# chintha/U-VIP-SLAM

Hardware: AMD Instinct MI355X
Metric: frames/sec ORB extract+match, 640x512 @1000 kp (higher is better)
Workload: dtype u8; 1 GPU; BASELINE.json configs[2]: 1xMI355X per rank, batch=256 synthetic 640x512 mono frames (+1 halo frame: the neighbouring rank's first), 1000 feats, 8 levels, fastTh 20, FullDetect extract + all-pairs 256-bit Hamming knn-2 of consecutive frames, HBM-resident I/O; batch_per_gpu=256, pipeline_depth=2, input_batches_in_rotation=4, fast_mode=adaptive

## Files before the change

u-vip-slam_amd/csrc/hamming.hip:

```cpp
#include "common.hpp"

namespace uvo {

constexpr int HM_TILE = 128;

__device__ __forceinline__ int popc256(const uint4& qa, const uint4& qb, const uint4& ta, const uint4& tb) {
  int d = __popc(qa.x ^ ta.x);
  d += __popc(qa.y ^ ta.y);
  d += __popc(qa.z ^ ta.z);
  d += __popc(qa.w ^ ta.w);
  d += __popc(qb.x ^ tb.x);
  d += __popc(qb.y ^ tb.y);
  d += __popc(qb.z ^ tb.z);
  d += __popc(qb.w ^ tb.w);
  return d;
}

__device__ __forceinline__ int clamp_count(int n, int cap) { return n < 0 ? 0 : (n > cap ? cap : n); }

__global__ __launch_bounds__(256) void k_knn2(const uint8_t* __restrict__ q, const int32_t* __restrict__ nq_arr, int nq_fixed, int q_stride,
                                              const uint8_t* __restrict__ t, const int32_t* __restrict__ nt_arr, int nt_fixed, int t_stride,
                                              const uint8_t* __restrict__ mask, int out_stride, int32_t* __restrict__ idx0,
                                              uint16_t* __restrict__ d0, int32_t* __restrict__ idx1, uint16_t* __restrict__ d1) {
  __shared__ uint4 s_t[HM_TILE * 2];
  const int pair = blockIdx.y;
  const int nq = nq_arr ? clamp_count(nq_arr[pair], q_stride < out_stride ? q_stride : out_stride) : nq_fixed;
  const int nt = nt_arr ? clamp_count(nt_arr[pair], t_stride < 65535 ? t_stride : 65535) : nt_fixed;
  const int qi = blockIdx.x * 256 + threadIdx.x;
  if (blockIdx.x * 256 >= nq) return;
  const uint4* Q = reinterpret_cast<const uint4*>(q + (int64_t)pair * q_stride * 32);
  const uint4* T = reinterpret_cast<const uint4*>(t + (int64_t)pair * t_stride * 32);
  const bool live = qi < nq;
  uint4 qa = make_uint4(0, 0, 0, 0), qb = qa;
  if (live) {
    qa = Q[2 * qi];
    qb = Q[2 * qi + 1];
  }
  uint32_t k0 = 0xFFFFFFFFu, k1 = 0xFFFFFFFFu;
  const uint8_t* mrow = mask ? mask + (int64_t)qi * nt : nullptr;
  for (int base = 0; base < nt; base += HM_TILE) {
    const int cnt = nt - base < HM_TILE ? nt - base : HM_TILE;
    __syncthreads();
    if ((int)threadIdx.x < 2 * cnt) s_t[threadIdx.x] = T[2 * base + threadIdx.x];
    __syncthreads();
    if (live) {
      for (int j = 0; j < cnt; ++j) {
        const uint32_t d = (uint32_t)popc256(qa, qb, s_t[2 * j], s_t[2 * j + 1]);
        uint32_t key = (d << 16) | (uint32_t)(base + j);
        if (mrow && !mrow[base + j]) key = 0xFFFFFFFFu;
        const uint32_t lo = min(k0, key);
        k1 = min(k1, max(k0, key));
        k0 = lo;
      }
    }
  }
  if (live) {
    const int64_t o = (int64_t)pair * out_stride + qi;
    idx0[o] = k0 == 0xFFFFFFFFu ? -1 : (int32_t)(k0 & 0xffffu);
    d0[o] = k0 == 0xFFFFFFFFu ? (uint16_t)0xFFFF : (uint16_t)(k0 >> 16);
    idx1[o] = k1 == 0xFFFFFFFFu ? -1 : (int32_t)(k1 & 0xffffu);
    d1[o] = k1 == 0xFFFFFFFFu ? (uint16_t)0xFFFF : (uint16_t)(k1 >> 16);
  }
}

typedef int v4i __attribute__((ext_vector_type(4)));
typedef int v16i __attribute__((ext_vector_type(16)));
constexpr int KM_ROW = 272;

__device__ __forceinline__ uint32_t spread4(uint32_t t) { return (__umul24(t & 0xfu, 0x00204081u)) & 0x01010101u; }
__device__ __forceinline__ v4i spread16(uint32_t x) {
  v4i r;
  r.x = (int)spread4(x), r.y = (int)spread4(x >> 4), r.z = (int)spread4(x >> 8), r.w = (int)spread4(x >> 12);
  return r;
}
__device__ __forceinline__ uint32_t spread4_ff(uint32_t t) {
  const uint32_t b = spread4(t);
  return (b << 8) - b;
}
__device__ __forceinline__ v4i spread16_ff(uint32_t x) {
  v4i r;
  r.x = (int)spread4_ff(x), r.y = (int)spread4_ff(x >> 4), r.z = (int)spread4_ff(x >> 8), r.w = (int)spread4_ff(x >> 12);
  return r;
}

__device__ __forceinline__ int med3_i32(int a, int b, int c) {
  int r;
  asm("v_med3_i32 %0, %1, %2, %3" : "=v"(r) : "v"(a), "v"(b), "v"(c));
  return r;
}

#ifndef UVO_OCC_KNN
#define UVO_OCC_KNN 6
#endif
__global__ __launch_bounds__(256, UVO_OCC_KNN) void k_knn2_mfma(const uint8_t* __restrict__ q, const int32_t* __restrict__ nq_arr, int nq_fixed, int q_stride,
                                                   const uint8_t* __restrict__ t, const int32_t* __restrict__ nt_arr, int nt_fixed, int t_stride,
                                                   int out_stride, int32_t* __restrict__ idx0, uint16_t* __restrict__ d0,
                                                   int32_t* __restrict__ idx1, uint16_t* __restrict__ d1) {
  __shared__ __attribute__((aligned(16))) uint8_t s_exp[32 * KM_ROW];
  __shared__ __attribute__((aligned(16))) int32_t s_key[32];
  const int pair = blockIdx.y;
  const int nq = nq_arr ? clamp_count(nq_arr[pair], q_stride < out_stride ? q_stride : out_stride) : nq_fixed;
  const int nt = nt_arr ? clamp_count(nt_arr[pair], t_stride < 65535 ? t_stride : 65535) : nt_fixed;
  if (blockIdx.x * 128 >= nq) return;
  const int lane = threadIdx.x & 63, wv = wave_in_block();
  const int r = lane & 31, h = lane >> 5;
  const int qi = blockIdx.x * 128 + wv * 32 + r;
  const uint32_t* Q = reinterpret_cast<const uint32_t*>(q + (int64_t)pair * q_stride * 32);
  const uint32_t* T = reinterpret_cast<const uint32_t*>(t + (int64_t)pair * t_stride * 32);
  v4i bq[8];
  int popq = 0;
#pragma unroll
  for (int s = 0; s < 8; ++s) {
    const uint32_t w = qi < nq ? Q[(int64_t)qi * 8 + s] : 0u;
    popq += __popc(w);
    bq[s] = spread16_ff(w >> (16 * h));
  }
  int k0 = 0x7fffffff, k1 = 0x7fffffff;
  const int erow = threadIdx.x >> 3, ec = threadIdx.x & 7;
  uint32_t wnext = erow < nt ? T[(int64_t)erow * 8 + ec] : 0u;
  for (int base = 0; base < nt; base += 32) {
    __syncthreads();
    {
      const int tr = base + erow;
      const uint32_t w = wnext;
      wnext = tr + 32 < nt ? T[(int64_t)(tr + 32) * 8 + ec] : 0u;
      v4i* dst = reinterpret_cast<v4i*>(s_exp + erow * KM_ROW + ec * 32);
      dst[0] = spread16(w), dst[1] = spread16(w >> 16);
      int pc = __popc(w);
      pc += __shfl_xor(pc, 1, 64);
      pc += __shfl_xor(pc, 2, 64);
      pc += __shfl_xor(pc, 4, 64);
      if (ec == 0) s_key[erow] = tr < nt ? ((pc << 16) | tr) : 0x7fff0000;
    }
    __syncthreads();
    v16i acc = {0, 0, 0, 0, 0, 0, 0, 0, 0, 0, 0, 0, 0, 0, 0, 0};
    const uint8_t* arow = s_exp + r * KM_ROW + 16 * h;
#pragma unroll
    for (int s = 0; s < 8; ++s) {
      const v4i a = *reinterpret_cast<const v4i*>(arow + 32 * s);
      acc = __builtin_amdgcn_mfma_i32_32x32x32_i8(a, bq[s], acc, 0, 0, 0);
    }
#pragma unroll
    for (int g = 0; g < 4; ++g) {
      const v4i kb = *reinterpret_cast<const v4i*>(&s_key[8 * g + 4 * h]);
      const int kbv[4] = {kb.x, kb.y, kb.z, kb.w};
#pragma unroll
      for (int e = 0; e < 4; ++e) {
        const int key = (int)(((uint32_t)acc[4 * g + e] << 17) + (uint32_t)kbv[e]);
        k1 = med3_i32(k0, k1, key);
        k0 = min(k0, key);
      }
    }
  }
  const int o0 = __shfl_xor(k0, 32, 64), o1 = __shfl_xor(k1, 32, 64);
  const int m0 = min(k0, o0), m1 = min(max(k0, o0), min(k1, o1));
  if (h == 0 && qi < nq) {
    const int64_t o = (int64_t)pair * out_stride + qi;
    const bool v0 = m0 < 0x7fff0000, v1 = m1 < 0x7fff0000;
    idx0[o] = v0 ? (m0 & 0xffff) : -1;
    d0[o] = v0 ? (uint16_t)((m0 >> 16) + popq) : (uint16_t)0xFFFF;
    idx1[o] = v1 ? (m1 & 0xffff) : -1;
    d1[o] = v1 ? (uint16_t)((m1 >> 16) + popq) : (uint16_t)0xFFFF;
  }
}

__global__ __launch_bounds__(256) void k_matrix(const uint8_t* __restrict__ q, int nq, const uint8_t* __restrict__ t, int nt,
                                                uint16_t* __restrict__ dist) {
  __shared__ uint4 s_t[HM_TILE * 2];
  const int qi = blockIdx.x * 256 + threadIdx.x;
  const uint4* Q = reinterpret_cast<const uint4*>(q);
  const uint4* T = reinterpret_cast<const uint4*>(t);
  const bool live = qi < nq;
  uint4 qa = make_uint4(0, 0, 0, 0), qb = qa;
  if (live) {
    qa = Q[2 * qi];
    qb = Q[2 * qi + 1];
  }
  const int base = blockIdx.y * HM_TILE;
  const int cnt = nt - base < HM_TILE ? nt - base : HM_TILE;
  if ((int)threadIdx.x < 2 * cnt) s_t[threadIdx.x] = T[2 * base + threadIdx.x];
  __syncthreads();
  if (!live) return;
  for (int j = 0; j < cnt; ++j) dist[(int64_t)qi * nt + base + j] = (uint16_t)popc256(qa, qb, s_t[2 * j], s_t[2 * j + 1]);
}

__global__ __launch_bounds__(256) void k_medoid(const uint8_t* __restrict__ desc, const int32_t* __restrict__ offsets, int32_t* __restrict__ best_idx,
                                                int32_t* __restrict__ best_median) {
  __shared__ uint32_t s_best;
  const int p = blockIdx.x;
  const int o0 = offsets[p], n = offsets[p + 1] - o0;
  if (threadIdx.x == 0) s_best = 0xFFFFFFFFu;
  __syncthreads();
  if (n > 0) {
    const uint4* D = reinterpret_cast<const uint4*>(desc + (int64_t)o0 * 32);
    const int k = (int)(0.5 * (n - 1));
    for (int i = threadIdx.x; i < n; i += 256) {
      const uint4 qa = D[2 * i], qb = D[2 * i + 1];
      int lo = 0, hi = 256;
      while (lo < hi) {
        const int mid = (lo + hi) >> 1;
        int c = 0;
        for (int j = 0; j < n; ++j) c += popc256(qa, qb, D[2 * j], D[2 * j + 1]) <= mid;
        if (c >= k + 1)
          hi = mid;
        else
          lo = mid + 1;
      }
      atomicMin(&s_best, ((uint32_t)lo << 16) | (uint32_t)i);
    }
  }
  __syncthreads();
  if (threadIdx.x == 0) {
    best_idx[p] = n > 0 ? (int32_t)(s_best & 0xffffu) : -1;
    best_median[p] = n > 0 ? (int32_t)(s_best >> 16) : -1;
  }
}

void launch_medoid(hipStream_t s, const uint8_t* d_desc, const int32_t* d_offsets, int npoints, int32_t* d_idx, int32_t* d_med) {
  hipLaunchKernelGGL(k_medoid, dim3(npoints), dim3(256), 0, s, d_desc, d_offsets, d_idx, d_med);
}

void launch_knn2(hipStream_t s, int pairs, int max_q, const uint8_t* d_q, const int32_t* d_nq, int nq_fixed, int q_stride, const uint8_t* d_t,
                 const int32_t* d_nt, int nt_fixed, int t_stride, const uint8_t* d_mask, int out_stride, int32_t* d_idx0, uint16_t* d_d0,
                 int32_t* d_idx1, uint16_t* d_d1) {
  if (!d_mask) {
    hipLaunchKernelGGL(k_knn2_mfma, dim3((max_q + 127) / 128, pairs), dim3(256), 0, s, d_q, d_nq, nq_fixed, q_stride, d_t, d_nt, nt_fixed, t_stride,
                       out_stride, d_idx0, d_d0, d_idx1, d_d1);
    return;
  }
  hipLaunchKernelGGL(k_knn2, dim3((max_q + 255) / 256, pairs), dim3(256), 0, s, d_q, d_nq, nq_fixed, q_stride, d_t, d_nt, nt_fixed, t_stride,
                     d_mask, out_stride, d_idx0, d_d0, d_idx1, d_d1);
}

void launch_matrix(hipStream_t s, const uint8_t* d_q, int nq, const uint8_t* d_t, int nt, uint16_t* d_dist) {
  hipLaunchKernelGGL(k_matrix, dim3((nq + 255) / 256, (nt + HM_TILE - 1) / HM_TILE), dim3(256), 0, s, d_q, nq, d_t, nt, d_dist);
}

}
```

Before: 313,100 frames/s.

## Fold Hamming key packing into MFMA accumulator init and process two query fragments

Adds a new int8 MFMA knn-2 kernel that seeds the accumulator with a packed key (target popcount shifted plus target index), so each output is already a sortable key. It pre-scales the bit-spread operands (shl 7 and shl 6) so the MFMA yields the -2·dot term inside the key, which removes the separate per-element shift/add after the MFMA. Each wave now handles two 32-query fragments to reuse the target tile loaded into LDS. It also prefetches the next target row into a register, and the launcher picks this path when the target count fits in 12 bits. The cost is more registers and lower declared occupancy, and the scaled int8 arithmetic has to stay within range.

Measured after the change: 312,700 frames/s. Within noise of the previous version (-0.1%).

```diff
diff --git a/u-vip-slam_amd/csrc/hamming.hip b/u-vip-slam_amd/csrc/hamming.hip
--- a/u-vip-slam_amd/csrc/hamming.hip
+++ b/u-vip-slam_amd/csrc/hamming.hip
@@ -86,6 +86,12 @@
 __device__ __forceinline__ int med3_i32(int a, int b, int c) {
   int r;
   asm("v_med3_i32 %0, %1, %2, %3" : "=v"(r) : "v"(a), "v"(b), "v"(c));
+  return r;
+}
+
+__device__ __forceinline__ int med3_i32_after(int a, int b, int c, int after) {
+  int r;
+  asm("v_med3_i32 %0, %1, %2, %3" : "=v"(r) : "v"(a), "v"(b), "v"(c), "v"(after));
   return r;
 }
 
@@ -161,6 +167,120 @@
     d0[o] = v0 ? (uint16_t)((m0 >> 16) + popq) : (uint16_t)0xFFFF;
     idx1[o] = v1 ? (m1 & 0xffff) : -1;
     d1[o] = v1 ? (uint16_t)((m1 >> 16) + popq) : (uint16_t)0xFFFF;
+  }
+}
+
+constexpr int KA_SHIFT = 12;
+constexpr int KA_S = 1 << KA_SHIFT;
+constexpr int KA_MAX_NT = KA_S;
+constexpr int KA_SENTINEL = 0x40000000;
+
+template <int SH>
+__device__ __forceinline__ v4i spread16_shl(uint32_t x) {
+  v4i r;
+  r.x = (int)(spread4(x) << SH), r.y = (int)(spread4(x >> 4) << SH), r.z = (int)(spread4(x >> 8) << SH), r.w = (int)(spread4(x >> 12) << SH);
+  return r;
+}
+
+#ifndef UVO_KNN_FRAGS
+#define UVO_KNN_FRAGS 2
+#endif
+#ifndef UVO_OCC_KNN_KEY
+#define UVO_OCC_KNN_KEY 4
+#endif
+template <int FRAGS>
+__global__ __launch_bounds__(256, UVO_OCC_KNN_KEY) void k_knn2_mfma_key(const uint8_t* __restrict__ q, const int32_t* __restrict__ nq_arr, int nq_fixed,
+                                                                            int q_stride, const uint8_t* __restrict__ t,
+                                                                            const int32_t* __restrict__ nt_arr, int nt_fixed, int t_stride, int out_stride,
+                                                                            int32_t* __restrict__ idx0, uint16_t* __restrict__ d0,
+                                                                            int32_t* __restrict__ idx1, uint16_t* __restrict__ d1) {
+  constexpr int QB = 128 * FRAGS;
+  __shared__ __attribute__((aligned(16))) uint8_t s_exp[32 * KM_ROW];
+  __shared__ __attribute__((aligned(16))) int32_t s_key[32];
+  const int pair = blockIdx.y;
+  const int nq = nq_arr ? clamp_count(nq_arr[pair], q_stride < out_stride ? q_stride : out_stride) : nq_fixed;
+  const int nt = nt_arr ? clamp_count(nt_arr[pair], t_stride < KA_MAX_NT ? t_stride : KA_MAX_NT) : nt_fixed;
+  if (blockIdx.x * QB >= nq) return;
+  const int lane = threadIdx.x & 63, wv = wave_in_block();
+  const int r = lane & 31, h = lane >> 5;
+  const int q0 = blockIdx.x * QB + wv * (32 * FRAGS) + r;
+  const uint32_t* Q = reinterpret_cast<const uint32_t*>(q + (int64_t)pair * q_stride * 32);
+  const uint32_t* T = reinterpret_cast<const uint32_t*>(t + (int64_t)pair * t_stride * 32);
+  v4i bq[FRAGS][8];
+  int popq[FRAGS], k0[FRAGS], k1[FRAGS];
+#pragma unroll
+  for (int f = 0; f < FRAGS; ++f) {
+    const int qi = q0 + 32 * f;
+    popq[f] = 0;
+#pragma unroll
+    for (int s = 0; s < 8; ++s) {
+      const uint32_t w = qi < nq ? Q[(int64_t)qi * 8 + s] : 0u;
+      popq[f] += __popc(w);
+      bq[f][s] = spread16_shl<7>(w >> (16 * h));
+    }
+    k0[f] = k1[f] = 0x7fffffff;
+  }
+  const int erow = threadIdx.x >> 3, ec = threadIdx.x & 7;
+  uint32_t wnext = erow < nt ? T[(int64_t)erow * 8 + ec] : 0u;
+  for (int base = 0; base < nt; base += 32) {
+    __syncthreads();
+    {
+      const int tr = base + erow;
+      const uint32_t w = wnext;
+      wnext = tr + 32 < nt ? T[(int64_t)(tr + 32) * 8 + ec] : 0u;
+      v4i* dst = reinterpret_cast<v4i*>(s_exp + erow * KM_ROW + ec * 32);
+      dst[0] = spread16_shl<6>(w), dst[1] = spread16_shl<6>(w >> 16);
+      int pc = __popc(w);
+      pc += __shfl_xor(pc, 1, 64);
+      pc += __shfl_xor(pc, 2, 64);
+      pc += __shfl_xor(pc, 4, 64);
+      if (ec == 0) s_key[erow] = tr < nt ? ((pc << KA_SHIFT) + tr) : KA_SENTINEL;
+    }
+    __syncthreads();
+    v16i acc[FRAGS];
+    const uint8_t* arow = s_exp + r * KM_ROW + 16 * h;
+    {
+      v16i c;
+#pragma unroll
+      for (int g = 0; g < 4; ++g) {
+        const v4i kb = *reinterpret_cast<const v4i*>(&s_key[8 * g + 4 * h]);
+        c[4 * g] = kb.x, c[4 * g + 1] = kb.y, c[4 * g + 2] = kb.z, c[4 * g + 3] = kb.w;
+      }
+      const v4i a = *reinterpret_cast<const v4i*>(arow);
+#pragma unroll
+      for (int f = 0; f < FRAGS; ++f) acc[f] = __builtin_amdgcn_mfma_i32_32x32x32_i8(a, bq[f][0], c, 0, 0, 0);
+    }
+#pragma unroll
+    for (int s = 1; s < 8; ++s) {
+      const v4i a = *reinterpret_cast<const v4i*>(arow + 32 * s);
+#pragma unroll
+      for (int f = 0; f < FRAGS; ++f) acc[f] = __builtin_amdgcn_mfma_i32_32x32x32_i8(a, bq[f][s], acc[f], 0, 0, 0);
+    }
+#pragma unroll
+    for (int f = 0; f < FRAGS; ++f) {
+#pragma unroll
+      for (int i = 0; i < 16; ++i) {
+        const int lo = min(k0[f], acc[f][i]);
+        k1[f] = med3_i32_after(k0[f], k1[f], acc[f][i], lo);
+        k0[f] = lo;
+      }
+    }
+  }
+#pragma unroll
+  for (int f = 0; f < FRAGS; ++f) {
+    const int o0 = __shfl_xor(k0[f], 32, 64), o1 = __shfl_xor(k1[f], 32, 64);
+    const int m0 = min(k0[f], o0), m1 = min(max(k0[f], o0), min(k1[f], o1));
+    const int qi = q0 + 32 * f;
+    if (h == 0 && qi < nq) {
+      const int64_t o = (int64_t)pair * out_stride + qi;
+      const bool v0 = m0 < KA_SENTINEL, v1 = m1 < KA_SENTINEL;
+      const uint32_t pq = (uint32_t)popq[f] << KA_SHIFT;
+      const int u0 = (int)((uint32_t)m0 + pq), u1 = (int)((uint32_t)m1 + pq);
+      idx0[o] = v0 ? (u0 & (KA_S - 1)) : -1;
+      d0[o] = v0 ? (uint16_t)(u0 >> KA_SHIFT) : (uint16_t)0xFFFF;
+      idx1[o] = v1 ? (u1 & (KA_S - 1)) : -1;
+      d1[o] = v1 ? (uint16_t)(u1 >> KA_SHIFT) : (uint16_t)0xFFFF;
+    }
   }
 }
 
@@ -224,6 +344,12 @@
                  const int32_t* d_nt, int nt_fixed, int t_stride, const uint8_t* d_mask, int out_stride, int32_t* d_idx0, uint16_t* d_d0,
                  int32_t* d_idx1, uint16_t* d_d1) {
   if (!d_mask) {
+    if ((d_nt ? t_stride : nt_fixed) <= KA_MAX_NT) {
+      constexpr int QB = 128 * UVO_KNN_FRAGS;
+      hipLaunchKernelGGL(k_knn2_mfma_key<UVO_KNN_FRAGS>, dim3((max_q + QB - 1) / QB, pairs), dim3(256), 0, s, d_q, d_nq, nq_fixed, q_stride, d_t,
+                         d_nt, nt_fixed, t_stride, out_stride, d_idx0, d_d0, d_idx1, d_d1);
+      return;
+    }
     hipLaunchKernelGGL(k_knn2_mfma, dim3((max_q + 127) / 128, pairs), dim3(256), 0, s, d_q, d_nq, nq_fixed, q_stride, d_t, d_nt, nt_fixed, t_stride,
                        out_stride, d_idx0, d_d0, d_idx1, d_d1);
     return;
```
